# YaqiangCao/cLoops

Measured on AMD Instinct MI355X. Metric: PETs clustered/sec (whole node) + wall-clock for mode-3 eps x minPts sweep, higher is better.
Workload: dtype int32; 1 GPU; synthetic-200M-23chr-mode3 (BASELINE.json configs[3]); variant=cDBSCAN2, pets=200000000, chromosomes=23, chained_cut=True, final_cut=3871, candidate_loops=3651369, parallelism=23 chromosomes LPT-sharded over 1 GPU(s)

## Files before the change

cloops_amd/csrc/cl_table.h:

```cpp
#pragma once
#include "cl_common.h"

struct Table {
    int* count; int* minx; int* maxx; int* miny; int* maxy;
    __device__ __forceinline__ cl_box get(int k) const
    {
        cl_box b; b.min_x = minx[k]; b.max_x = maxx[k]; b.min_y = miny[k]; b.max_y = maxy[k]; b.count = count[k];
        return b;
    }
};

__device__ __forceinline__ int wave_min_i(int v) { return dpp_reduce_wave(v, OpMin()); }
__device__ __forceinline__ int wave_max_i(int v) { return dpp_reduce_wave(v, OpMax()); }

#ifndef TAB_BITS
#define TAB_BITS 9
#endif
#define TAB_H (1 << TAB_BITS)
struct TableLds { int key[TAB_H], cnt[TAB_H], mnx[TAB_H], mxx[TAB_H], mny[TAB_H], mxy[TAB_H]; };

__device__ __forceinline__ void table_lds_init(TableLds& h)
{
    for (int k = threadIdx.x; k < TAB_H; k += blockDim.x) {
        h.key[k] = -1; h.cnt[k] = 0; h.mnx[k] = INT_MAX; h.mxx[k] = INT_MIN; h.mny[k] = INT_MAX; h.mxy[k] = INT_MIN;
// ... 9 lines not shown
        h = (h + 1) & (TAB_H - 1);
    }
    return -1;
}
__device__ __forceinline__ int wave_shr1(int v) { return __builtin_amdgcn_update_dpp(v, v, 0x138, 0xf, 0xf, false); }
struct WaveRuns { int dist; bool last; };
__device__ __forceinline__ WaveRuns wave_runs(int v)
{
    const int lane = threadIdx.x & 63;
    const int prev = wave_shr1(v);
    const unsigned long long B = __ballot(lane == 0 || prev != v);
    const int start = 63 - __clzll((long long)(B & (~0ull >> (63 - lane))));
    WaveRuns r;
    r.dist = lane - start;
    r.last = lane == 63 || ((B >> (lane + 1)) & 1ull);
    return r;
}
#define SEG_STEP(ctrl, rowmask, cond, ...) seg_step_values<ctrl, rowmask>((cond), __VA_ARGS__)
template <int CTRL, int ROWMASK>
__device__ __forceinline__ void seg_step_values(bool take, int& mn0, int& mx0, int& mn1, int& mx1)
{
    const int a = min(mn0, __builtin_amdgcn_update_dpp(mn0, mn0, CTRL, ROWMASK, 0xf, false));
    const int b = max(mx0, __builtin_amdgcn_update_dpp(mx0, mx0, CTRL, ROWMASK, 0xf, false));
    const int c = min(mn1, __builtin_amdgcn_update_dpp(mn1, mn1, CTRL, ROWMASK, 0xf, false));
    const int d = max(mx1, __builtin_amdgcn_update_dpp(mx1, mx1, CTRL, ROWMASK, 0xf, false));
    mn0 = take ? a : mn0; mx0 = take ? b : mx0; mn1 = take ? c : mn1; mx1 = take ? d : mx1;
}
template <int CTRL, int ROWMASK>
__device__ __forceinline__ void seg_step_min(bool take, int& m)
{
    const int a = min(m, __builtin_amdgcn_update_dpp(m, m, CTRL, ROWMASK, 0xf, false));
    m = take ? a : m;
}
__device__ __forceinline__ void table_accumulate(const Table& t, TableLds& h, int lab, int x, int y)
{
    if (!__any(lab >= 0)) return;
    const int lane = threadIdx.x & 63;
    const WaveRuns r = wave_runs(lab);
    int mnx = x, mxx = x, mny = y, mxy = y;
    SEG_STEP(0x111, 0xf, r.dist >= 1, mnx, mxx, mny, mxy);
    SEG_STEP(0x112, 0xf, r.dist >= 2, mnx, mxx, mny, mxy);
    SEG_STEP(0x114, 0xf, r.dist >= 4, mnx, mxx, mny, mxy);
    SEG_STEP(0x118, 0xf, r.dist >= 8, mnx, mxx, mny, mxy);
    SEG_STEP(0x142, 0xa, r.dist > (lane & 15), mnx, mxx, mny, mxy);
    SEG_STEP(0x143, 0xc, r.dist > (lane & 31), mnx, mxx, mny, mxy);
    if (r.last && lab >= 0) {
        const int cm = r.dist + 1;
        const int sl = tab_slot(h.key, lab);
        if (sl >= 0) {
            atomicAdd(&h.cnt[sl], cm);
            atomicMin(&h.mnx[sl], mnx); atomicMax(&h.mxx[sl], mxx);
            atomicMin(&h.mny[sl], mny); atomicMax(&h.mxy[sl], mxy);
        } else {
            atomicAdd(&t.count[lab], cm);
            atomicMin(&t.minx[lab], mnx); atomicMax(&t.maxx[lab], mxx);
            atomicMin(&t.miny[lab], mny); atomicMax(&t.maxy[lab], mxy);
        }
    }
}
__device__ __forceinline__ void table_flush(const Table& t, TableLds& h)
{
    __syncthreads();
    for (int k = threadIdx.x; k < TAB_H; k += blockDim.x) {
        if (h.key[k] < 0) continue;
        const int L = h.key[k];
        atomicAdd(&t.count[L], h.cnt[k]);
// ... 7 lines not shown
```

cloops_amd/csrc/k_lists.hip:

```cpp
#include "cl_chrom.h"

#ifdef CLOOPS_DEVEL
#define L_ABL(bit) (g.dbg2 & (bit))
#else
#define L_ABL(bit) 0
#endif
#ifdef CLOOPS_DEVEL
__device__ unsigned long long g_lstat[32];
__device__ __forceinline__ void lstat_add(int slot, int v)
{
    int t = v;
    for (int o = 32; o > 0; o >>= 1) t += __shfl_down(t, o);
    if ((threadIdx.x & 63) == 0 && t) atomicAdd(&g_lstat[slot], (unsigned long long)t);
}
extern "C" void cl_debug_lstats(unsigned long long* out)
{
    (void)hipDeviceSynchronize();
    (void)hipMemcpyFromSymbol(out, HIP_SYMBOL(g_lstat), sizeof(g_lstat));
    unsigned long long z[32] = {0};
    (void)hipMemcpyToSymbol(HIP_SYMBOL(g_lstat), z, sizeof(z));
}
#define LSTAT_ON (g.dbg2 & (1 << 30))
#define LSTAT(slot, v) do { if (LSTAT_ON) lstat_add((slot), (v)); } while (0)
#else
// ... 377 lines not shown
        const int fin = min(m, lmin[l_hlast - t0]);
        if (threadIdx.x == 0) lmin[l_hlast - t0] = fin;
        for (int j = tend + (int)threadIdx.x; j < jend; j += 64) bkey[j] = fin;
    }
    __syncthreads();
#pragma unroll
    for (int u = 0; u < 8; ++u) {
        const int i = t0 + u * 256 + (int)threadIdx.x;
        if (i < npos && pos[u] >= t0) bkey[i] = lmin[pos[u] - t0];
    }
}

__global__ void __launch_bounds__(256)
k_words_to_base(GridParams g, int npos, const int* __restrict__ bsp, const int4* __restrict__ tab, const int* __restrict__ poff,
                const int* __restrict__ run_words, int* __restrict__ words)
{
    const int b = blockIdx.x * blockDim.x + threadIdx.x;
    if (b >= npos) return;
    const int st = min(bsp[b] >> g.rbits, g.S);
    const int4 t = tab[st];
    if (b < t.x) return;
    int w = run_words[b - poff[st]];
    if (w < 0 && ((unsigned)w & K2H_NONE) != K2H_NONE) {
        const int da = (int)((unsigned)w & K2H_MASK) + t.z, db = (int)(((unsigned)w >> K2H_BITS) & K2H_MASK) + tab[min(st + 1, g.S)].z;
        const bool ok = (da < (int)K2H_MASK) & (db < (int)K2H_MASK);
        w = (int)(((unsigned)w & ~K2H_NONE) | (ok ? ((unsigned)da | ((unsigned)db << K2H_BITS)) : K2H_NONE));
    }
    words[b] = w;
}

template <bool CUT, bool BAND>
__global__ void __launch_bounds__(256)
k_classify_q(GridParams g, int npos, int thr, int bandq, const int* __restrict__ bq, const int* __restrict__ words,
             const int* __restrict__ band, unsigned long long* __restrict__ cmask, unsigned long long* __restrict__ wmask,
             int* __restrict__ cgloc, int* __restrict__ wgloc, int* __restrict__ bsum, unsigned long long* __restrict__ sup)
{
    __shared__ int l_cc[LG], l_wc[LG];
    const int nblk = (int)gridDim.x, blk = (int)blockIdx.x;
    const int t0 = blk * LT;
    const int lane = threadIdx.x & 63, wv = threadIdx.x >> 6;
    int q[8], w[8];
#pragma unroll
    for (int u = 0; u < 8; ++u) { const int b = t0 + u * 256 + (int)threadIdx.x; q[u] = (CUT && b < npos) ? bq[b] : INT_MAX; }
#pragma unroll
    for (int u = 0; u < 8; ++u) {
        const int b = t0 + u * 256 + (int)threadIdx.x;
        const bool alive = b < npos && (!CUT || q[u] >= thr);
        const int* src = (BAND && q[u] < bandq) ? band : words;
        w[u] = alive ? src[b] : 0;
    }
#pragma unroll
    for (int u = 0; u < 8; ++u) {
        const bool core = cw_core(w[u], g.minPts) && w[u] != 0;
        const bool walk = !core && cw_count(w[u]) > 1;
        const unsigned long long cb = __ballot(core), wb = __ballot(walk);
        const int k = u * 4 + wv, gidx = (t0 >> 6) + k;
        if (lane == 0) { cmask[gidx] = cb; wmask[gidx] = wb; l_cc[k] = __popcll(cb); l_wc[k] = __popcll(wb); }
    }
    if (blk == nblk - 1 && threadIdx.x == 0) {
        const int ge = nblk * LG;
        cmask[ge] = 0ull; wmask[ge] = 0ull; cgloc[ge] = 0; wgloc[ge] = 0;
    }
    __syncthreads();
    if (threadIdx.x < 64) {
        const int k = lane & 31;
        const int v = lane < 32 ? l_cc[k] : l_wc[k];
        int incl = v;
#pragma unroll
        for (int d = 1; d < 32; d <<= 1) { const int t = __shfl_up(incl, d, 32); incl += k >= d ? t : 0; }
        (lane < 32 ? cgloc : wgloc)[(t0 >> 6) + k] = incl - v;
        const int totC = __shfl(incl, 31), totW = __shfl(incl, 63);
        if (threadIdx.x == 0 && !L_ABL(1 << 18)) {
            bsum[blk] = totC; bsum[nblk + 1 + blk] = totW;
            const unsigned long long both = (unsigned long long)(unsigned)totC | ((unsigned long long)(unsigned)totW << 32);
            if (both) atomicAdd(&sup[blk >> 4], both);
        }
    }
}

template <bool V2, bool CUT, bool BAND>
__global__ void __launch_bounds__(256)
k_make_lists_q(GridParams g, int npos, int bandq, const int* __restrict__ bq, const int* __restrict__ bsp, const u32* __restrict__ brow,
               const int* __restrict__ bkey, const int2* __restrict__ fix, const int* __restrict__ words, const int* __restrict__ band,
               const unsigned long long* __restrict__ cmask, const unsigned long long* __restrict__ wmask, const int* __restrict__ cgloc,
               const int* __restrict__ wgloc, const int* __restrict__ bsum, const unsigned long long* __restrict__ sup,
               int* __restrict__ cgrank, int* __restrict__ wgrank, int2* __restrict__ cpair, int* __restrict__ cpos,
               int* __restrict__ ckey, int2* __restrict__ wpair, int* __restrict__ wpos, int* __restrict__ wenc, int* __restrict__ lcnt,
               int* __restrict__ parent )
{
    __shared__ int l_red[2][4];
    const int nblk = (int)gridDim.x, blk = (int)blockIdx.x;
    const int t0 = blk * LT;
    const int lane = threadIdx.x & 63, wv = threadIdx.x >> 6;
    unsigned long long cbv[8], wbv[8];
    int cgv[8], wgv[8], q[8], sp[8], aux[8];
#pragma unroll
    for (int u = 0; u < 8; ++u) {
        const int gidx = (t0 >> 6) + u * 4 + wv;
        cbv[u] = cmask[gidx]; wbv[u] = wmask[gidx];
        cgv[u] = cgloc[gidx]; wgv[u] = wgloc[gidx];
        const int b = t0 + u * 256 + (int)threadIdx.x;
        q[u] = b < npos ? bq[b] : 0; sp[u] = b < npos ? bsp[b] : 0;
    }
    {
        int2 fx[8];
#pragma unroll
        for (int u = 0; u < 8; ++u) {
            const int b = t0 + u * 256 + (int)threadIdx.x;
// ... 125 lines not shown
    }
}

#define LU_MAXB 4
__device__ __forceinline__ int lower_bound_pairs(const int2* __restrict__ pv, int lo, int hi, int val)
{
    while (hi - lo > 4) {
        const int qq = (hi - lo) >> 2;
        const int m1 = lo + qq, m2 = m1 + qq, m3 = m2 + qq;
        const int v1 = pv[m1].x, v2 = pv[m2].x, v3 = pv[m3].x;
        if (v1 >= val) hi = m1;
        else if (v2 >= val) { lo = m1 + 1; hi = m2; }
        else if (v3 >= val) { lo = m2 + 1; hi = m3; }
        else lo = m3 + 1;
    }
    while (lo < hi && pv[lo].x < val) ++lo;
    return lo;
}

struct HeadReset { int* compkey; int* ncore; int* bsize; int* usize; int* state; };
template <int NT, int HALO, bool FUSE>
__global__ void __launch_bounds__(256)
k_union_c(GridParams g, int ntiles, const int* __restrict__ lcnt, const int2* __restrict__ cpair, int* chainid,
          const int* __restrict__ cstrip, int* cskip, int* parent, HeadReset hr, int* __restrict__ ckey_prune ,
          int* __restrict__ ovlist, int* __restrict__ counters)
{
    constexpr int WIN = NT + HALO;
    constexpr int NCH = WIN / 64;
    __shared__ int2 lw[WIN];
    __shared__ int lx[WIN];
    __shared__ int lend[WIN];
    __shared__ unsigned long long l_ob[FUSE ? NCH : 1];
    __shared__ int l_found;
    const int C = lcnt[0];
    const int tile = ltile_of_block(blockIdx.x);
    const int t0 = tile * NT;
    if (tile >= ntiles || t0 >= C) return;
    const int base = t0 - HALO;
    const int lane = threadIdx.x & 63;
    const int nmask = ~(g.peps - 1);
    if (FUSE && threadIdx.x == 0) l_found = -1;
    int pf_tb[NT / 256], pf_b[NT / 256];
    {
        constexpr int SU = (WIN + 255) / 256;
        static_assert(WIN % 64 == 0, "whole waves in the last staging round");
        int2 mv[SU], pvl[SU];
#pragma unroll
        for (int u = 0; u < SU; ++u) {
            const int gi = base + u * 256 + (int)threadIdx.x;
            const bool in = gi >= 0 && gi < C && u * 256 + (int)threadIdx.x < WIN;
            mv[u] = in ? cpair[gi] : (gi < 0 ? make_int2(0, INT_MIN) : make_int2(INT_MAX, INT_MAX));
            pvl[u] = (FUSE && lane == 0 && gi > 0 && gi < C) ? cpair[gi - 1] : make_int2(0, 0);
        }
        if (HALO % 256 == 0) {
#pragma unroll
            for (int u2 = 0; u2 < NT / 256; ++u2) {
                const int gi = t0 + u2 * 256 + (int)threadIdx.x;
                const int s = mv[HALO / 256 + u2].y >> g.rbits;
                const bool ok = gi < C && s > 0;
                pf_tb[u2] = ok ? cstrip[s - 1] : 0; pf_b[u2] = ok ? cstrip[s] : 0;
            }
        }
#pragma unroll
        for (int u = 0; u < SU; ++u) {
            const int k = u * 256 + (int)threadIdx.x, gi = base + k;
            if (k >= WIN) continue;
            const bool in = gi >= 0 && gi < C;
            const int2 me = mv[u];
            lw[k] = me;
            if (!FUSE) { lx[k] = in ? chainid[gi] : -1; lend[k] = in ? cskip[gi] : 0; }
            else {
                int2 pv = make_int2(wave_shr1(me.x), wave_shr1(me.y));
                if (lane == 0 && gi > 0 && gi < C) pv = pvl[u];
                const bool o = gi <= 0 ? gi == 0 : (gi >= C || (pv.y & nmask) != (me.y & nmask) || pv.x < me.x - g.eps);
                const unsigned long long ob = __ballot(o);
                if (lane == 0) l_ob[k >> 6] = ob;
            }
        }
    }
    __syncthreads();
    if (FUSE) {
        if (threadIdx.x < 64 && base > 0 && !(l_ob[0] & 1ull)) {
            int found = -1;
            for (int k0 = base - 64; found < 0; k0 -= 64) {
                const int j = k0 + lane;
                bool o = false;
                if (j >= 0) {
                    const int2 a = cpair[j];
                    const int2 b = j > 0 ? cpair[j - 1] : make_int2(0, INT_MIN);
                    o = j == 0 || (b.y & nmask) != (a.y & nmask) || b.x < a.x - g.eps;
                }
                const unsigned long long bal = __ballot(o);
                if (bal) found = k0 + 63 - __clzll((long long)bal);
            }
            if (lane == 0) l_found = found;
        }
        __syncthreads();
        for (int k = threadIdx.x; k < WIN; k += 256) {
            const int ch = k >> 6, gi = base + k;
            const unsigned long long ob = l_ob[ch];
            const unsigned long long upto = ob & (~0ull >> (63 - lane));
            int head;
            if (upto) head = base + ch * 64 + 63 - __clzll((long long)upto);
            else {
                head = l_found;
                for (int c2 = ch - 1; c2 >= 0; --c2) { const unsigned long long o2 = l_ob[c2]; if (o2) { head = base + c2 * 64 + 63 - __clzll((long long)o2); break; } }
            }
            const unsigned long long above = lane == 63 ? 0ull : (ob & (~0ull << (lane + 1)));
            int skip;
            if (above) skip = base + ch * 64 + __ffsll((long long)above) - 1;
            else {
                skip = base + WIN;
                for (int c2 = ch + 1; c2 < NCH; ++c2) { const unsigned long long o2 = l_ob[c2]; if (o2) { skip = base + c2 * 64 + __ffsll((long long)o2) - 1; break; } }
            }
            const bool in = gi >= 0 && gi < C;
            lx[k] = in ? head : -1;
            lend[k] = in ? min(skip, C) : 0;
            if (in && k >= HALO) {
                chainid[gi] = head;
                cskip[gi] = min(skip, C);
                if (head == gi) { hr.compkey[gi] = INT_MAX; hr.ncore[gi] = 0; hr.bsize[gi] = 0; hr.usize[gi] = 0; hr.state[gi] = ST_LIVE; }
                if (ckey_prune && gi > 0) {
                    const int2 me = lw[k], pv = lw[k - 1];
                    if ((pv.y & nmask) == (me.y & nmask) && div_eps(g, pv.x) == div_eps(g, me.x)) ckey_prune[gi] = INT_MAX;
                }
            }
        }
        __syncthreads();
    }
    const int wbeg = max(base, 0);
    LdsPairs w; w.a = lw; w.base = base;
    constexpr int PER = NT / 256;
#pragma unroll 1
    for (int u = 0; u < PER; ++u) {
        const int i = t0 + u * 256 + (int)threadIdx.x;
        const bool in = i < C;
        int Bs[LU_MAXB];
#pragma unroll
        for (int k = 0; k < LU_MAXB; ++k) Bs[k] = -1;
        int nb = 0;
        int A = -1;
#ifdef CLOOPS_DEVEL
        int st_it = 0, st_touch = 0, st_glb = 0, st_jump = 0;
#endif
        if (in) {
            const int2 me = lw[i - base];
            A = lx[i - base];
            const int s = me.y >> g.rbits;
            int tb, b;
            if (HALO % 256 == 0) { tb = u == 0 ? pf_tb[0] : pf_tb[NT / 256 - 1]; b = u == 0 ? pf_b[0] : pf_b[NT / 256 - 1]; }
            else { tb = s > 0 ? cstrip[s - 1] : 0; b = s > 0 ? cstrip[s] : 0; }
            if (tb < b) {
                const int qlo = me.x - g.eps, qhi = me.x + g.eps;
                const int T = me.y - g.peps;
                if (tb < wbeg && wbeg < b && lw[wbeg - base].x < qlo) tb = wbeg;
                auto touch = [&](int B) {
                    bool seen = false;
#pragma unroll
                    for (int k = 0; k < LU_MAXB; ++k) seen |= (Bs[k] == B);
                    if (seen) return;
#ifdef CLOOPS_DEVEL
                    ++st_touch;
#endif
                    if (nb < LU_MAXB) {
#pragma unroll
                        for (int k = 0; k < LU_MAXB; ++k) if (k == nb) Bs[k] = B;
                        ++nb;
                    } else {
                        uf_unite(parent, A, B);
                    }
                };
                if (L_ABL(1 << 17)) tb = b;
                if (tb >= b) { }
                else if (tb >= wbeg && b - tb <= 2047) {
                    const int len = b - tb;
                    int j;
                    if (len <= 31) j = lds_lower_bound8<5>(w, tb, b, qlo);
                    else if (len <= 63) j = lds_lower_bound8<6>(w, tb, b, qlo);
                    else if (len <= 255) j = lds_lower_bound8<8>(w, tb, b, qlo);
                    else j = lds_lower_bound8<11>(w, tb, b, qlo);
                    if (L_ABL(1 << 16)) j = b;
                    while (j < b) {
#ifdef CLOOPS_DEVEL
                        ++st_it;
#endif
                        int2 cv[4];
#pragma unroll
                        for (int k = 0; k < 4; ++k) cv[k] = lw[min(j + k, b - 1) - base];
                        int f = 4; bool fh = false;
#pragma unroll
                        for (int k = 3; k >= 0; --k) {
                            const bool bey = (j + k >= b) | (cv[k].x > qhi);
                            const bool hit = cv[k].y >= T;
                            if (bey | hit) { f = k; fh = hit & !bey; }
                        }
                        if (f == 4) { j += 4; continue; }
                        if (!fh) break;
                        const int idx = j + f - base;
                        touch(lx[idx]);
#ifdef CLOOPS_DEVEL
                        ++st_jump;
#endif
                        j = lend[idx];
                    }
                } else if (FUSE) {
                    ovlist[atomicAdd(&counters[CTR_NOVF], 1)] = i;
                } else {
#ifdef CLOOPS_DEVEL
                    ++st_glb;
#endif
                    int k = lower_bound_pairs(cpair, tb, b, qlo);
                    while (k < b) {
                        int2 cv[4]; int bv[4];
#pragma unroll
                        for (int e = 0; e < 4; ++e) { const int idx = min(k + e, b - 1); cv[e] = cpair[idx]; bv[e] = chainid[idx]; }
                        int next = k + 4;
                        bool stop = false;
#pragma unroll
                        for (int e = 0; e < 4; ++e) {
                            if (stop || k + e >= b) continue;
                            if (cv[e].x > qhi) { stop = true; next = b; continue; }
                            if (cv[e].y >= T) {
                                touch(bv[e]);
                                stop = true;
                                next = cskip[min(k + e, b - 1)];
                            }
                        }
                        k = next;
                    }
                }
            }
        }
        int st_un = 0;
#pragma unroll
        for (int k = 0; k < LU_MAXB; ++k) {
            const int B = Bs[k];
            unsigned long long pending = __ballot(B >= 0);
            bool rep = false;
            while (pending) {
                const int leader = __ffsll((long long)pending) - 1;
                const int LA = __builtin_amdgcn_readlane(A, leader), LB = __builtin_amdgcn_readlane(B, leader);
                const unsigned long long m = __ballot(B >= 0 && A == LA && B == LB);
                if (lane == leader) rep = true;
                pending &= ~m;
            }
            if (rep && !L_ABL(1 << 15)) { uf_unite(parent, A, B); ++st_un; }
        }
#ifdef CLOOPS_DEVEL
        LSTAT(12, in ? 1 : 0); LSTAT(13, st_it); LSTAT(14, st_touch); LSTAT(15, st_un); LSTAT(16, st_glb); LSTAT(17, st_jump);
        { int mx = st_it; for (int o2 = 32; o2 > 0; o2 >>= 1) mx = max(mx, __shfl_down(mx, o2)); if (lane == 0 && LSTAT_ON) { atomicAdd(&g_lstat[18], (unsigned long long)mx); atomicAdd(&g_lstat[19], 1ull); }
          if (LSTAT_ON && st_it > 2) atomicAdd(&g_lstat[20], 1ull); if (LSTAT_ON && st_it > 4) atomicAdd(&g_lstat[21], 1ull); if (LSTAT_ON && st_it > 8) atomicAdd(&g_lstat[22], 1ull); }
#else
        (void)st_un;
#endif
    }
}

__global__ void k_prep_c(GridParams g, const int* __restrict__ lcnt, const int* __restrict__ strip_start,
                         const unsigned long long* __restrict__ cmask, const int* __restrict__ cgrank, int* __restrict__ cstrip,
                         int* __restrict__ sup, int nsup2, int* __restrict__ parent )
{
    const int C = lcnt[0];
    const int u = blockIdx.x * blockDim.x + threadIdx.x;
    if (parent && u < C) parent[u] = u;
    if (u <= g.S + 1) {
        const int M = strip_start[g.S];
        const int p = u <= g.S ? strip_start[u] : M;
        cstrip[u] = p < M ? core_rank(cmask, cgrank, p) : C;
    }
    if (u < nsup2) sup[u] = 0;
}
__global__ void k_union_overflow(GridParams g, const int* __restrict__ counters, const int* __restrict__ ovlist, const int2* __restrict__ cpair,
                                 const int* __restrict__ chainid, const int* __restrict__ cstrip, const int* __restrict__ cskip, int* parent)
{
    const int nov = counters[CTR_NOVF];
    for (int t = blockIdx.x * blockDim.x + threadIdx.x; t < nov; t += gridDim.x * blockDim.x) {
        const int i = ovlist[t];
        const int2 me = cpair[i];
        const int A = chainid[i];
        const int s = me.y >> g.rbits;
        if (s <= 0) continue;
        const int tb = cstrip[s - 1], b = cstrip[s];
// ... 829 lines not shown
    c->l_sup_dirty = true;
    launch_classify(c, g, nblk, b);
    launch_make_lists(c, g, nblk, b, L);
    fuse_knob(c);
    if (c->fuse_chains)
        hipLaunchKernelGGL(k_prep_c, dim3(nblocks(std::max(std::max(nm, g.S + 2), b.nsup2))), dim3(TPB), 0, c->stream, g, (const int*)L.lcnt, (const int*)c->w_strip,
                           (const unsigned long long*)L.cmask, (const int*)L.cgrank, L.cstrip, b.sup, b.nsup2, c->parent.as<int>());
#ifdef CLOOPS_DEVEL
    else
    hipLaunchKernelGGL(k_chain_c, dim3(nblocks(nm, 256 * CH_PER)), dim3(256), 0, c->stream, g, L.lcnt, (const int2*)L.cpair, c->chainflag.as<int>(),
                       c->parent.as<int>(), c->compkey.as<int>(), c->ncore.as<int>(), c->bsize.as<int>(), c->usize.as<int>(), c->state.as<int>(),
                       c->cellfirst.as<int>() , (const int*)c->w_strip, L.cmask, L.cgrank, L.cstrip, b.sup, b.nsup2, (int*)nullptr);
#else
    { }
#endif
    L.npos = nm; L.pstrip = c->w_strip;
    *out = L;
    HIP_TRY(hipGetLastError());
    c->l_sup_dirty = false;
    return CL_OK;
}

int lists_base_keys(cl_chrom* c, const GridParams& g)
{
    const int n = (int)c->n;
    int rc = c->bkey.ensure((size_t)n * 4);
    if (rc) return rc;
    hipLaunchKernelGGL(k_base_keys, dim3(nblocks(n, LT)), dim3(256), 0, c->stream, g, n, (const int*)(c->bq.as<int>() + SORT_PAD),
                       (const int*)(c->bsp.as<int>() + SORT_PAD), (const u32*)c->brow.as<u32>(), c->bkey.as<int>());
    HIP_TRY(hipGetLastError());
    return CL_OK;
}

int lists_build_base(cl_chrom* c, const GridParams& g, int nm, ListRun* out)
{
    fuse_knob(c);
    const int n = (int)c->n;
    ListBufs b;
    int rc = list_bufs(c, g, n, &b);
    if (rc) return rc;
    const int nblk = nblocks(n, LT);
    const bool v2 = g.variant == CL_VARIANT_CDBSCAN2;
    ListRun L{};
    list_views(c, b, &L);
    L.npos = n; L.pstrip = c->bstrip.as<int>();
    unsigned long long* sup64 = (unsigned long long*)b.sup;
    const int nsup_ints = 2 * (nblk / 16 + 2);
    if (c->l_sup_dirty) HIP_TRY(hipMemsetAsync(b.sup, 0, (size_t)std::max(nsup_ints, b.nsup2) * 4, c->stream));
    c->l_sup_dirty = true;
    const int* bq = c->bq.as<int>() + SORT_PAD;
    const int* bsp = c->bsp.as<int>() + SORT_PAD;
    const u32* brow = c->brow.as<u32>();
    c->srow = c->brow.as<u32>();
    const int* words = c->rc_cnt.as<int>();
    const int* band = c->cnt.as<int>();
    const int thr = c->l4_cut ? g.cut - g.V0 : INT_MIN;
    const int bandq = c->ws.bandq;
#define LCQ_ARGS g, n, thr, bandq, bq, words, band, b.cmask, b.wmask, b.cgloc, b.wgloc, b.bsum, sup64
    if (!c->l4_cut) hipLaunchKernelGGL((k_classify_q<false, false>), dim3(nblk), dim3(256), 0, c->stream, LCQ_ARGS);
    else if (c->l4_band) hipLaunchKernelGGL((k_classify_q<true, true>), dim3(nblk), dim3(256), 0, c->stream, LCQ_ARGS);
    else hipLaunchKernelGGL((k_classify_q<true, false>), dim3(nblk), dim3(256), 0, c->stream, LCQ_ARGS);
#undef LCQ_ARGS
#define LMQ_ARGS g, n, bandq, bq, bsp, brow, (const int*)c->bkey.as<int>(), (const int2*)c->l_fix.as<int2>(), words, band, (const unsigned long long*)b.cmask,                  \
                 (const unsigned long long*)b.wmask, (const int*)b.cgloc, (const int*)b.wgloc, (const int*)b.bsum, (const unsigned long long*)sup64, b.cgrank, b.wgrank, L.cpair,  \
                 c->run_rows ? L.cpos : (int*)nullptr, L.ckey, L.wpair, L.wpos, L.wenc, b.lcnt, c->fuse_chains ? c->parent.as<int>() : (int*)nullptr
    if (v2) {
        if (!c->l4_cut) hipLaunchKernelGGL((k_make_lists_q<true, false, false>), dim3(nblk), dim3(256), 0, c->stream, LMQ_ARGS);
        else if (c->l4_band) hipLaunchKernelGGL((k_make_lists_q<true, true, true>), dim3(nblk), dim3(256), 0, c->stream, LMQ_ARGS);
        else hipLaunchKernelGGL((k_make_lists_q<true, true, false>), dim3(nblk), dim3(256), 0, c->stream, LMQ_ARGS);
    } else {
        if (c->l4_band) hipLaunchKernelGGL((k_make_lists_q<false, true, true>), dim3(nblk), dim3(256), 0, c->stream, LMQ_ARGS);
        else hipLaunchKernelGGL((k_make_lists_q<false, false, false>), dim3(nblk), dim3(256), 0, c->stream, LMQ_ARGS);
    }
#undef LMQ_ARGS
    fuse_knob(c);
    if (c->fuse_chains)
        hipLaunchKernelGGL(k_prep_c, dim3(nblocks(std::max(g.S + 2, std::max(nsup_ints, b.nsup2)))), dim3(TPB), 0, c->stream, g, (const int*)L.lcnt,
                           (const int*)L.pstrip, (const unsigned long long*)L.cmask, (const int*)L.cgrank, L.cstrip, b.sup, std::max(nsup_ints, b.nsup2), (int*)nullptr);
#ifdef CLOOPS_DEVEL
    else
    hipLaunchKernelGGL(k_chain_c, dim3(nblocks(nm, 256 * CH_PER)), dim3(256), 0, c->stream, g, L.lcnt, (const int2*)L.cpair, c->chainflag.as<int>(),
                       c->parent.as<int>(), c->compkey.as<int>(), c->ncore.as<int>(), c->bsize.as<int>(), c->usize.as<int>(), c->state.as<int>(),
                       c->cellfirst.as<int>() , L.pstrip, L.cmask, L.cgrank, L.cstrip, b.sup, std::max(nsup_ints, b.nsup2), v2 ? L.ckey : (int*)nullptr);
#else
    { }
#endif
    *out = L;
    HIP_TRY(hipGetLastError());
    c->l_sup_dirty = false;
    return CL_OK;
}

int lists_words_to_base(cl_chrom* c, const GridParams& g)
{
    const int n = (int)c->n;
// ... 182 lines not shown
    HIP_TRY(hipMemsetAsync(p + o_sup, 0, nsup * 8, c->stream));
    hipLaunchKernelGGL(k_rowmask_count, dim3((unsigned)ntile), dim3(256), 0, c->stream, (int)n, (const int*)sl.labels.as<int>(), (unsigned long long*)p,
                       (int*)(p + o_tsum), (unsigned long long*)(p + o_sup));
    hipLaunchKernelGGL(k_rowmask_write, dim3((unsigned)ntile), dim3(256), 0, c->stream, (int)n, (const int*)sl.labels.as<int>(), (const unsigned long long*)p,
                       (const int*)(p + o_tsum), (const unsigned long long*)(p + o_sup), (int*)(p + o_lab), (long long)c->mask_cap, total);
    HIP_TRY(hipGetLastError());
    return CL_OK;
}

#ifdef CLOOPS_DEVEL
extern "C" int cl_debug_time_lists(cl_chrom* c, int which, int reps, float* ms_out)
{
    if (!c || !ms_out || c->dbg_nm <= 0) return fail(CL_ERR_ARG, "cl_debug_time_lists: no rotated run on this handle");
    HIP_TRY(hipSetDevice(c->device));
    GridParams g = c->dbg_g;
    { const char* e = getenv("CLOOPS_DBG2"); g.dbg2 = e ? atoi(e) : 0; }
    const int nm = c->dbg_nm;
    ListBufs b;
    int rc = list_bufs(c, g, nm, &b);
    if (rc) return rc;
    const int nblk = nblocks(nm, LT);
    ListRun L{};
    list_views(c, b, &L);
    hipEvent_t e0, e1;
    HIP_TRY(hipEventCreate(&e0)); HIP_TRY(hipEventCreate(&e1));
    HIP_TRY(hipStreamSynchronize(c->stream));
    HIP_TRY(hipEventRecord(e0, c->stream));
    for (int r = 0; r < reps; ++r) {
        if (which == 0) {
            HIP_TRY(hipMemsetAsync(b.sup, 0, (size_t)b.nsup2 * 4, c->stream));
            launch_classify(c, g, nblk, b);
        } else if (which == 1) {
            launch_make_lists(c, g, nblk, b, L);
        } else if (which == 6 || which == 7) {
            const int n = (int)c->n;
            ListBufs bb;
            if ((rc = list_bufs(c, g, n, &bb))) return rc;
            const int nb4 = nblocks(n, LT);
            unsigned long long* sup64 = (unsigned long long*)bb.sup;
            const int* bq = c->bq.as<int>() + SORT_PAD; const int* bsp = c->bsp.as<int>() + SORT_PAD;
            const int thr = g.cut - g.V0, bandq = c->ws.bandq;
            if (which == 6) {
                HIP_TRY(hipMemsetAsync(bb.sup, 0, (size_t)2 * (nb4 / 16 + 2) * 4, c->stream));
                hipLaunchKernelGGL((k_classify_q<true, true>), dim3(nb4), dim3(256), 0, c->stream, g, n, thr, bandq, bq, (const int*)c->rc_cnt.as<int>(), (const int*)c->cnt.as<int>(),
                                   bb.cmask, bb.wmask, bb.cgloc, bb.wgloc, bb.bsum, sup64);
            } else {
                hipLaunchKernelGGL((k_make_lists_q<true, true, true>), dim3(nb4), dim3(256), 0, c->stream, g, n, bandq, bq, bsp, (const u32*)c->brow.as<u32>(), (const int*)c->bkey.as<int>(),
                                   (const int2*)c->l_fix.as<int2>(), (const int*)c->rc_cnt.as<int>(), (const int*)c->cnt.as<int>(), (const unsigned long long*)bb.cmask,
                                   (const unsigned long long*)bb.wmask, (const int*)bb.cgloc, (const int*)bb.wgloc, (const int*)bb.bsum, (const unsigned long long*)sup64, bb.cgrank, bb.wgrank,
                                   L.cpair, (int*)nullptr, L.ckey, L.wpair, L.wpos, L.wenc, bb.lcnt, (int*)nullptr);
            }
        } else if (which == 4 || which == 3 || which == 5) {
            ListRun L2 = L;
            c->run_level = c->traversal >= 4 ? 4 : 3;
            if (c->run_level == 4) { ListBufs bb; if ((rc = list_bufs(c, g, (int)c->n, &bb))) return rc; list_views(c, bb, &L2); L2.npos = (int)c->n; L2.pstrip = c->bstrip.as<int>(); }
            else { L2.npos = nm; L2.pstrip = c->w_strip; }
            if (which == 4) { if ((rc = lists_border(c, g, nm, L2))) return rc; }
            else if (which == 3) {
                ListBufs bb; if ((rc = list_bufs(c, g, c->run_level == 4 ? (int)c->n : nm, &bb))) return rc;
                fuse_knob(c);
                if (c->fuse_chains)
                    hipLaunchKernelGGL(k_prep_c, dim3(nblocks(std::max(nm, g.S + 2))), dim3(TPB), 0, c->stream, g, (const int*)L2.lcnt, (const int*)L2.pstrip,
                                       (const unsigned long long*)L2.cmask, (const int*)L2.cgrank, L2.cstrip, bb.sup, 2, c->parent.as<int>());
#ifdef CLOOPS_DEVEL
                else
                hipLaunchKernelGGL(k_chain_c, dim3(nblocks(nm, 256 * CH_PER)), dim3(256), 0, c->stream, g, L2.lcnt, (const int2*)L2.cpair, c->chainflag.as<int>(),
                                   c->parent.as<int>(), c->compkey.as<int>(), c->ncore.as<int>(), c->bsize.as<int>(), c->usize.as<int>(), c->state.as<int>(),
                                   c->cellfirst.as<int>(), L2.pstrip, L2.cmask, L2.cgrank, L2.cstrip, bb.sup, 2, (int*)nullptr);
#else
    { }
#endif
                HIP_TRY(hipMemsetAsync(c->counters.p, 0, 64, c->stream));
                if ((rc = lists_union_flatten(c, g, nm, L2))) return rc;
            } else { if ((rc = lists_final(c, g, nm, L2, false, c->counters.as<int>() + 40))) return rc; }
        } else return fail(CL_ERR_ARG, "cl_debug_time_lists: kernel not supported on its own");
    }
    HIP_TRY(hipEventRecord(e1, c->stream));
    HIP_TRY(hipEventSynchronize(e1));
    if (which == 1 || which == 7) HIP_TRY(hipMemsetAsync(b.sup, 0, c->l_blk.bytes - 64, c->stream));
    float ms = 0.f;
    (void)hipEventElapsedTime(&ms, e0, e1);
    *ms_out = ms / (float)std::max(1, reps);
    (void)hipEventDestroy(e0); (void)hipEventDestroy(e1);
    return CL_OK;
}
#endif
```

Baseline: 15.51 billion PETs/s.

## Compact union-search work list in LDS and skip dominated cores

Adds a pre-pass in k_union_c that decides for each core in the tile whether a neighbour search is needed. It packs the search bounds into a compact LDS work list, and waves then iterate densely over that list instead of over every tile slot. In the fused path it also uses segmented wave prefix/suffix minima to skip cores dominated by neighbours in the same cell. This reduces divergence and idle lanes in the search loop, at the cost of an extra pass, LDS space, atomics, and a possible correctness risk from the domination skip.

```diff
diff --git a/cloops_amd/csrc/cl_table.h b/cloops_amd/csrc/cl_table.h
--- a/cloops_amd/csrc/cl_table.h
+++ b/cloops_amd/csrc/cl_table.h
@@ -65,6 +65,45 @@
     const int a = min(m, __builtin_amdgcn_update_dpp(m, m, CTRL, ROWMASK, 0xf, false));
     m = take ? a : m;
 }
+__device__ __forceinline__ int wave_shl1(int v) { return __builtin_amdgcn_update_dpp(v, v, 0x130, 0xf, 0xf, false); }
+struct WaveSegs { int dist, rdist; };
+__device__ __forceinline__ WaveSegs wave_segs(bool open)
+{
+    const int lane = threadIdx.x & 63;
+    const unsigned long long B = __ballot(open) | 1ull;
+    const int start = 63 - __clzll((long long)(B & (~0ull >> (63 - lane))));
+    const unsigned long long above = lane == 63 ? 0ull : (B & (~0ull << (lane + 1)));
+    const int end = above ? __ffsll((long long)above) - 1 : 64;
+    WaveSegs r;
+    r.dist = lane - start;
+    r.rdist = end - 1 - lane;
+    return r;
+}
+__device__ __forceinline__ int seg_prefix_min(const WaveSegs& w, int m)
+{
+    const int lane = threadIdx.x & 63;
+    seg_step_min<0x111, 0xf>(w.dist >= 1, m);
+    seg_step_min<0x112, 0xf>(w.dist >= 2, m);
+    seg_step_min<0x114, 0xf>(w.dist >= 4, m);
+    seg_step_min<0x118, 0xf>(w.dist >= 8, m);
+    seg_step_min<0x142, 0xa>(w.dist > (lane & 15), m);
+    seg_step_min<0x143, 0xc>(w.dist > (lane & 31), m);
+    return m;
+}
+__device__ __forceinline__ int seg_suffix_min(const WaveSegs& w, int m)
+{
+    const int lane = threadIdx.x & 63;
+    seg_step_min<0x101, 0xf>(w.rdist >= 1, m);
+    seg_step_min<0x102, 0xf>(w.rdist >= 2, m);
+    seg_step_min<0x104, 0xf>(w.rdist >= 4, m);
+    seg_step_min<0x108, 0xf>(w.rdist >= 8, m);
+#pragma unroll
+    for (int r = 3; r >= 1; --r) {
+        const int v = __builtin_amdgcn_readlane(m, 16 * r);
+        m = ((lane >> 4) == r - 1 && w.rdist > 15 - (lane & 15)) ? min(m, v) : m;
+    }
+    return m;
+}
 __device__ __forceinline__ void table_accumulate(const Table& t, TableLds& h, int lab, int x, int y)
 {
     if (!__any(lab >= 0)) return;
diff --git a/cloops_amd/csrc/k_lists.hip b/cloops_amd/csrc/k_lists.hip
--- a/cloops_amd/csrc/k_lists.hip
+++ b/cloops_amd/csrc/k_lists.hip
@@ -666,6 +666,10 @@
     __shared__ int lend[WIN];
     __shared__ unsigned long long l_ob[FUSE ? NCH : 1];
     __shared__ int l_found;
+    __shared__ unsigned lsv[NT];
+    __shared__ int l_ns;
+    constexpr int PER = NT / 256;
+    static_assert(NT <= 512 && WIN <= 1024, "a list entry packs the core's offset in the tile and its window in the staged range");
     const int C = lcnt[0];
     const int tile = ltile_of_block(blockIdx.x);
     const int t0 = tile * NT;
@@ -673,8 +677,8 @@
     const int base = t0 - HALO;
     const int lane = threadIdx.x & 63;
     const int nmask = ~(g.peps - 1);
-    if (FUSE && threadIdx.x == 0) l_found = -1;
-    int pf_tb[NT / 256], pf_b[NT / 256];
+    if (threadIdx.x == 0) { l_found = -1; l_ns = 0; }
+    int pf_tb[PER], pf_b[PER];
     {
         constexpr int SU = (WIN + 255) / 256;
         static_assert(WIN % 64 == 0, "whole waves in the last staging round");
@@ -713,6 +717,49 @@
         }
     }
     __syncthreads();
+    const int wbeg = max(base, 0);
+    {
+        int tbv[PER], bv[PER];
+#pragma unroll
+        for (int u2 = 0; u2 < PER; ++u2) {
+            if (HALO % 256 == 0) { tbv[u2] = pf_tb[u2]; bv[u2] = pf_b[u2]; }
+            else {
+                const int k = HALO + u2 * 256 + (int)threadIdx.x;
+                const int s = lw[k].y >> g.rbits;
+                const bool ok = base + k < C && s > 0;
+                tbv[u2] = ok ? cstrip[s - 1] : 0; bv[u2] = ok ? cstrip[s] : 0;
+            }
+        }
+#pragma unroll
+        for (int u2 = 0; u2 < PER; ++u2) {
+            const int k = HALO + u2 * 256 + (int)threadIdx.x, gi = base + k;
+            const bool in = gi < C;
+            const int2 me = lw[k];
+            bool dom = false;
+            if (FUSE) {
+                const int px = wave_shr1(me.x), py = wave_shr1(me.y);
+                const WaveSegs sg = wave_segs(!in || (py & nmask) != (me.y & nmask) || div_eps(g, px) != div_eps(g, me.x));
+                const int fmin = wave_shr1(seg_prefix_min(sg, me.y)), bmin = wave_shl1(seg_suffix_min(sg, me.y));
+                dom = sg.dist >= 1 && fmin <= me.y && sg.rdist >= 1 && bmin < me.y;
+            }
+            int tb = tbv[u2];
+            const int b = bv[u2];
+            bool srch = in && !dom && tb < b && !L_ABL(1 << 17);
+            if (srch && tb < wbeg && wbeg < b && lw[wbeg - base].x < me.x - g.eps) tb = wbeg;
+            const bool staged = tb >= wbeg && b - tb <= 2047;
+            LSTAT(12, in ? 1 : 0); LSTAT(23, srch ? 1 : 0);
+            if (FUSE && srch && !staged) {
+                ovlist[atomicAdd(&counters[CTR_NOVF], 1)] = gi;
+                srch = false;
+            }
+            const unsigned long long sb = __ballot(srch);
+            int wb = 0;
+            if (lane == 0 && sb) wb = atomicAdd(&l_ns, __popcll(sb));
+            wb = __builtin_amdgcn_readfirstlane(wb);
+            if (srch) lsv[wb + lane_rank(sb)] = (unsigned)(k - HALO) | (staged ? ((unsigned)(tb - base) << 9) | ((unsigned)(b - base) << 19) : 0x80000000u);
+        }
+    }
+    if (!FUSE) __syncthreads();
     if (FUSE) {
         if (threadIdx.x < 64 && base > 0 && !(l_ob[0] & 1ull)) {
             int found = -1;
@@ -762,13 +809,11 @@
         }
         __syncthreads();
     }
-    const int wbeg = max(base, 0);
     LdsPairs w; w.a = lw; w.base = base;
-    constexpr int PER = NT / 256;
+    const int ns = l_ns;
 #pragma unroll 1
-    for (int u = 0; u < PER; ++u) {
-        const int i = t0 + u * 256 + (int)threadIdx.x;
-        const bool in = i < C;
+    for (int n0 = (int)threadIdx.x - lane; n0 < ns; n0 += 256) {
+        const bool in = n0 + lane < ns;
         int Bs[LU_MAXB];
 #pragma unroll
         for (int k = 0; k < LU_MAXB; ++k) Bs[k] = -1;
@@ -778,16 +823,14 @@
         int st_it = 0, st_touch = 0, st_glb = 0, st_jump = 0;
 #endif
         if (in) {
-            const int2 me = lw[i - base];
-            A = lx[i - base];
-            const int s = me.y >> g.rbits;
-            int tb, b;
-            if (HALO % 256 == 0) { tb = u == 0 ? pf_tb[0] : pf_tb[NT / 256 - 1]; b = u == 0 ? pf_b[0] : pf_b[NT / 256 - 1]; }
-            else { tb = s > 0 ? cstrip[s - 1] : 0; b = s > 0 ? cstrip[s] : 0; }
-            if (tb < b) {
+            const unsigned ent = lsv[n0 + lane];
+            const int k0 = HALO + (int)(ent & 511u);
+            const bool staged = !(ent >> 31);
+            const int2 me = lw[k0];
+            A = lx[k0];
+            {
                 const int qlo = me.x - g.eps, qhi = me.x + g.eps;
                 const int T = me.y - g.peps;
-                if (tb < wbeg && wbeg < b && lw[wbeg - base].x < qlo) tb = wbeg;
                 auto touch = [&](int B) {
                     bool seen = false;
 #pragma unroll
@@ -804,9 +847,8 @@
                         uf_unite(parent, A, B);
                     }
                 };
-                if (L_ABL(1 << 17)) tb = b;
-                if (tb >= b) { }
-                else if (tb >= wbeg && b - tb <= 2047) {
+                if (staged) {
+                    const int tb = base + (int)((ent >> 9) & 1023u), b = base + (int)((ent >> 19) & 1023u);
                     const int len = b - tb;
                     int j;
                     if (len <= 31) j = lds_lower_bound8<5>(w, tb, b, qlo);
@@ -837,12 +879,12 @@
 #endif
                         j = lend[idx];
                     }
-                } else if (FUSE) {
-                    ovlist[atomicAdd(&counters[CTR_NOVF], 1)] = i;
-                } else {
+                } else if (!FUSE) {
 #ifdef CLOOPS_DEVEL
                     ++st_glb;
 #endif
+                    const int s = me.y >> g.rbits;
+                    const int tb = cstrip[s - 1], b = cstrip[s];
                     int k = lower_bound_pairs(cpair, tb, b, qlo);
                     while (k < b) {
                         int2 cv[4]; int bv[4];
@@ -881,7 +923,7 @@
             if (rep && !L_ABL(1 << 15)) { uf_unite(parent, A, B); ++st_un; }
         }
 #ifdef CLOOPS_DEVEL
-        LSTAT(12, in ? 1 : 0); LSTAT(13, st_it); LSTAT(14, st_touch); LSTAT(15, st_un); LSTAT(16, st_glb); LSTAT(17, st_jump);
+        LSTAT(13, st_it); LSTAT(14, st_touch); LSTAT(15, st_un); LSTAT(16, st_glb); LSTAT(17, st_jump);
         { int mx = st_it; for (int o2 = 32; o2 > 0; o2 >>= 1) mx = max(mx, __shfl_down(mx, o2)); if (lane == 0 && LSTAT_ON) { atomicAdd(&g_lstat[18], (unsigned long long)mx); atomicAdd(&g_lstat[19], 1ull); }
           if (LSTAT_ON && st_it > 2) atomicAdd(&g_lstat[20], 1ull); if (LSTAT_ON && st_it > 4) atomicAdd(&g_lstat[21], 1ull); if (LSTAT_ON && st_it > 8) atomicAdd(&g_lstat[22], 1ull); }
 #else
```

Result: no change. 15.46 billion PETs/s (-0.3%).

## Split walker classification into a pass that drops walkers seeing no core

Applied to the files above, without the earlier changes.

Core classification and walker classification now run as two kernels. The new walker kernel marks a border candidate as a walker only if a core point lies within eps in an adjacent strip. It checks this with a shared-memory copy of the core bitmask plus a halo, and falls back to a global bitmask search when the halo is not enough. The aim is to shrink the walker lists that later list-building and union stages must process, at the cost of an extra launch, extra bitmask/bq/bsp reads and possible divergence on the slow path.

```diff
diff --git a/cloops_amd/csrc/k_lists.hip b/cloops_amd/csrc/k_lists.hip
--- a/cloops_amd/csrc/k_lists.hip
+++ b/cloops_amd/csrc/k_lists.hip
@@ -433,10 +433,10 @@
 template <bool CUT, bool BAND>
 __global__ void __launch_bounds__(256)
 k_classify_q(GridParams g, int npos, int thr, int bandq, const int* __restrict__ bq, const int* __restrict__ words,
-             const int* __restrict__ band, unsigned long long* __restrict__ cmask, unsigned long long* __restrict__ wmask,
-             int* __restrict__ cgloc, int* __restrict__ wgloc, int* __restrict__ bsum, unsigned long long* __restrict__ sup)
-{
-    __shared__ int l_cc[LG], l_wc[LG];
+             const int* __restrict__ band, unsigned long long* __restrict__ cmask, int* __restrict__ cgloc, int* __restrict__ bsum,
+             unsigned long long* __restrict__ sup)
+{
+    __shared__ int l_cc[LG];
     const int nblk = (int)gridDim.x, blk = (int)blockIdx.x;
     const int t0 = blk * LT;
     const int lane = threadIdx.x & 63, wv = threadIdx.x >> 6;
@@ -453,28 +453,224 @@
 #pragma unroll
     for (int u = 0; u < 8; ++u) {
         const bool core = cw_core(w[u], g.minPts) && w[u] != 0;
-        const bool walk = !core && cw_count(w[u]) > 1;
-        const unsigned long long cb = __ballot(core), wb = __ballot(walk);
+        const unsigned long long cb = __ballot(core);
         const int k = u * 4 + wv, gidx = (t0 >> 6) + k;
-        if (lane == 0) { cmask[gidx] = cb; wmask[gidx] = wb; l_cc[k] = __popcll(cb); l_wc[k] = __popcll(wb); }
+        if (lane == 0) { cmask[gidx] = cb; l_cc[k] = __popcll(cb); }
     }
     if (blk == nblk - 1 && threadIdx.x == 0) {
         const int ge = nblk * LG;
-        cmask[ge] = 0ull; wmask[ge] = 0ull; cgloc[ge] = 0; wgloc[ge] = 0;
+        cmask[ge] = 0ull; cgloc[ge] = 0;
     }
     __syncthreads();
-    if (threadIdx.x < 64) {
-        const int k = lane & 31;
-        const int v = lane < 32 ? l_cc[k] : l_wc[k];
+    if (threadIdx.x < 32) {
+        const int k = lane;
+        const int v = l_cc[k];
         int incl = v;
 #pragma unroll
         for (int d = 1; d < 32; d <<= 1) { const int t = __shfl_up(incl, d, 32); incl += k >= d ? t : 0; }
-        (lane < 32 ? cgloc : wgloc)[(t0 >> 6) + k] = incl - v;
-        const int totC = __shfl(incl, 31), totW = __shfl(incl, 63);
+        cgloc[(t0 >> 6) + k] = incl - v;
+        const int totC = __shfl(incl, 31, 32);
         if (threadIdx.x == 0 && !L_ABL(1 << 18)) {
-            bsum[blk] = totC; bsum[nblk + 1 + blk] = totW;
-            const unsigned long long both = (unsigned long long)(unsigned)totC | ((unsigned long long)(unsigned)totW << 32);
-            if (both) atomicAdd(&sup[blk >> 4], both);
+            bsum[blk] = totC;
+            if (totC) atomicAdd(&sup[blk >> 4], (unsigned long long)(unsigned)totC);
+        }
+    }
+}
+
+__device__ __forceinline__ int first_core_in(const unsigned long long* __restrict__ cmask, int from, int end)
+{
+    if (from >= end) return end;
+    int gi = from >> 6;
+    const int ge = (end - 1) >> 6;
+    unsigned long long m = cmask[gi] & ~low_mask(from & 63);
+    while (!m && gi < ge) m = cmask[++gi];
+    return m ? min((gi << 6) + __ffsll((long long)m) - 1, end) : end;
+}
+__device__ __forceinline__ int last_core_in(const unsigned long long* __restrict__ cmask, int beg, int to)
+{
+    if (to <= beg) return -1;
+    int gi = (to - 1) >> 6;
+    const int gb = beg >> 6;
+    unsigned long long m = cmask[gi] & (((to - 1) & 63) == 63 ? ~0ull : low_mask(to & 63));
+    while (!m && gi > gb) m = cmask[--gi];
+    if (!m) return -1;
+    const int p = (gi << 6) + 63 - __clzll((long long)m);
+    return p >= beg ? p : -1;
+}
+__device__ __forceinline__ int lower_bound_q(const int* __restrict__ bq, int lo, int hi, int val)
+{
+    while (lo < hi) { const int mid = (int)(((unsigned)lo + (unsigned)hi) >> 1); if (bq[mid] < val) lo = mid + 1; else hi = mid; }
+    return lo;
+}
+__device__ __noinline__ bool walker_sees_core(int rbits, int S, int eps, int b, int q, int sp, int w, const int* __restrict__ bq,
+                                              const int* __restrict__ bsp, const int* __restrict__ bstrip, const unsigned long long* __restrict__ cmask)
+{
+    const int s = min(sp >> rbits, S - 1), peps = 1 << rbits;
+    const int qlo = q - eps, qhi = q + eps;
+    const int pbeg = sp & ~(peps - 1), pend = pbeg + peps, pend2 = pend + peps;
+    const int sb0 = bstrip[s], sb1 = bstrip[s + 1], sb2 = bstrip[min(s + 2, S)];
+    const unsigned enc = lh_pack(w, 0, 0);
+    const bool hinted = enc != LH_NONE;
+    bool keep = false;
+    const int pl = last_core_in(cmask, sb0, b);
+    if (pl >= 0) keep = (bsp[pl] >= pbeg) & (bq[pl] >= qlo);
+    if (!keep) {
+        const int pr = first_core_in(cmask, b + 1, sb1);
+        if (pr < sb1) keep = (bsp[pr] < pend) & (bq[pr] <= qhi);
+    }
+    if (!keep && s > 0) {
+        const int pa = hinted ? b - (int)(enc & 0xffffu) : lower_bound_q(bq, bstrip[s - 1], sb0, qlo);
+        const int pc = first_core_in(cmask, max(pa, 0), b);
+        if (pc < b) keep = (bsp[pc] < pbeg) & (bq[pc] <= qhi);
+    }
+    if (!keep) {
+        const int pb = hinted ? b + (int)(enc >> 16) : lower_bound_q(bq, sb1, sb2, qlo);
+        const int pc = first_core_in(cmask, pb, sb2);
+        if (pc < sb2) keep = (bsp[pc] < pend2) & (bq[pc] <= qhi);
+    }
+    return keep;
+}
+#define WQ_HALO 4096
+#define WQ_NW ((LT + 2 * WQ_HALO) / 64)
+template <bool CUT, bool BAND>
+__global__ void __launch_bounds__(256)
+k_walkers_q(GridParams g, int npos, int thr, int bandq, const int* __restrict__ bq, const int* __restrict__ bsp,
+            const int* __restrict__ bstrip, const int* __restrict__ words, const int* __restrict__ band,
+            const unsigned long long* __restrict__ cmask, unsigned long long* __restrict__ wmask, int* __restrict__ wgloc,
+            int* __restrict__ bsum, unsigned long long* __restrict__ sup)
+{
+    static_assert(WQ_NW <= 192 && (int)K2H_MASK < WQ_HALO, "three words of non-empty bits; a hint stays inside the halo");
+    __shared__ int l_wc[LG];
+    __shared__ unsigned long long l_cm[WQ_NW];
+    __shared__ unsigned long long l_nz[3];
+    const int nblk = (int)gridDim.x, blk = (int)blockIdx.x;
+    const int t0 = blk * LT;
+    const int lane = threadIdx.x & 63, wv = threadIdx.x >> 6;
+    const int gw0 = (t0 - WQ_HALO) >> 6;
+    const int wlo = max(t0 - WQ_HALO, 0), wend = min(t0 + LT + WQ_HALO, nblk * LT);
+    int q[8], w[8], sp[8];
+#pragma unroll
+    for (int u = 0; u < 8; ++u) { const int b = t0 + u * 256 + (int)threadIdx.x; q[u] = b < npos ? bq[b] : INT_MAX; }
+    {
+        const int k = (int)threadIdx.x, gw = gw0 + k;
+        const unsigned long long v = (k < WQ_NW && gw >= 0 && gw < nblk * LG) ? cmask[gw] : 0ull;
+        if (k < WQ_NW) l_cm[k] = v;
+        const unsigned long long nz = __ballot(v != 0ull);
+        if (lane == 0 && wv < 3) l_nz[wv] = nz;
+    }
+    const int sp_lo = bsp[wlo], sp_hi = bsp[min(wend, npos) - 1];
+    const bool at_front = wlo == 0, at_back = wend >= npos;
+#pragma unroll
+    for (int u = 0; u < 8; ++u) {
+        const int b = t0 + u * 256 + (int)threadIdx.x;
+        const bool alive = b < npos && (!CUT || q[u] >= thr);
+        const int* src = (BAND && q[u] < bandq) ? band : words;
+        w[u] = alive ? src[b] : 0;
+    }
+    int ncls = 0;
+#pragma unroll
+    for (int u = 0; u < 8; ++u) {
+        const int b = t0 + u * 256 + (int)threadIdx.x;
+        const bool core = cw_core(w[u], g.minPts) && w[u] != 0;
+        const bool walk = !core && cw_count(w[u]) > 1;
+        sp[u] = walk ? bsp[b] : 0;
+        if (!walk) w[u] = 0;
+        ncls += walk ? 1 : 0;
+    }
+    LSTAT(23, ncls);
+    (void)ncls;
+    __syncthreads();
+    auto next_core = [&](int from, int end) -> int {
+        if (from >= end) return -1;
+        int k = (from >> 6) - gw0;
+        if (k >= WQ_NW) return -1;
+        unsigned long long m = l_cm[k] & ~low_mask(from & 63);
+        if (!m) {
+            const int kk = k + 1;
+            int k2 = -1;
+#pragma unroll
+            for (int j = 2; j >= 0; --j) {
+                const unsigned long long mm = l_nz[j] & (j == (kk >> 6) ? ~low_mask(kk & 63) : (j > (kk >> 6) ? ~0ull : 0ull));
+                if (mm) k2 = j * 64 + __ffsll((long long)mm) - 1;
+            }
+            if (k2 < 0) return -1;
+            k = k2; m = l_cm[k2];
+        }
+        const int p = ((gw0 + k) << 6) + __ffsll((long long)m) - 1;
+        return p < end ? p : -1;
+    };
+    auto prev_core = [&](int beg, int to) -> int {
+        if (to <= beg) return -1;
+        const int last = to - 1;
+        int k = (last >> 6) - gw0;
+        unsigned long long m = l_cm[k] & ((last & 63) == 63 ? ~0ull : low_mask((last & 63) + 1));
+        if (!m) {
+            const int kk = k - 1;
+            if (kk < 0) return -1;
+            int k2 = -1;
+#pragma unroll
+            for (int j = 0; j < 3; ++j) {
+                const unsigned long long upto = (kk & 63) == 63 ? ~0ull : low_mask((kk & 63) + 1);
+                const unsigned long long mm = l_nz[j] & (j == (kk >> 6) ? upto : (j < (kk >> 6) ? ~0ull : 0ull));
+                if (mm) k2 = j * 64 + 63 - __clzll((long long)mm);
+            }
+            if (k2 < 0) return -1;
+            k = k2; m = l_cm[k2];
+        }
+        const int p = ((gw0 + k) << 6) + 63 - __clzll((long long)m);
+        return p >= beg ? p : -1;
+    };
+    int slow = 0;
+#pragma unroll
+    for (int u = 0; u < 8; ++u) {
+        const int b = t0 + u * 256 + (int)threadIdx.x;
+        const bool walk = w[u] != 0;
+        bool keep = false;
+        if (__ballot(walk)) {
+            const unsigned enc = lh_pack(w[u], 0, 0);
+            const bool hinted = enc != LH_NONE;
+            const int pa = b - (int)(enc & 0xffffu), pb = b + (int)(enc >> 16);
+            const int pl = walk ? prev_core(wlo, b) : -1;
+            const int pr = walk ? next_core(b + 1, wend) : -1;
+            const int pc = (walk && hinted && pa >= wlo) ? next_core(pa, b) : -1;
+            const int pd = (walk && hinted) ? next_core(pb, wend) : -1;
+            const int bs = min(b, npos - 1);
+            const int il = pl >= 0 ? pl : bs, ir = pr >= 0 ? pr : bs, ic = pc >= 0 ? pc : bs, id = pd >= 0 ? pd : bs;
+            const int ql = bq[il], qr = bq[ir], qc = bq[ic], qd = bq[id];
+            const int sl = bsp[il], sr = bsp[ir], sc = bsp[ic], sd = bsp[id];
+            const int qlo = q[u] - g.eps, qhi = q[u] + g.eps;
+            const int pbeg = sp[u] & ~(g.peps - 1), pend = pbeg + g.peps, pend2 = pend + g.peps;
+            keep = walk & (((pl >= 0) & (sl >= pbeg) & (ql >= qlo)) | ((pr >= 0) & (sr < pend) & (qr <= qhi)) |
+                           ((pc >= 0) & (sc < pbeg) & (qc <= qhi)) | ((pd >= 0) & (sd < pend2) & (qd <= qhi)));
+            const bool open_l = (pl < 0) & !(at_front | (sp_lo < pbeg));
+            const bool open_r = (pr < 0) & !(at_back | (sp_hi >= pend));
+            const bool open_d = (pd < 0) & !(at_back | (sp_hi >= pend2));
+            if (walk & !keep & (!hinted | (pa < wlo) | open_l | open_r | open_d)) slow |= 1 << u;
+        }
+        if (__any(slow >> u & 1)) {
+            if (slow >> u & 1) keep = walker_sees_core(g.rbits, g.S, g.eps, b, q[u], sp[u], w[u], bq, bsp, bstrip, cmask);
+            LSTAT(24, slow >> u & 1);
+        }
+        const unsigned long long wb = __ballot(keep);
+        const int k = u * 4 + wv, gidx = (t0 >> 6) + k;
+        if (lane == 0) { wmask[gidx] = wb; l_wc[k] = __popcll(wb); }
+    }
+    if (blk == nblk - 1 && threadIdx.x == 0) {
+        const int ge = nblk * LG;
+        wmask[ge] = 0ull; wgloc[ge] = 0;
+    }
+    __syncthreads();
+    if (threadIdx.x < 32) {
+        const int k = lane;
+        const int v = l_wc[k];
+        int incl = v;
+#pragma unroll
+        for (int d = 1; d < 32; d <<= 1) { const int t = __shfl_up(incl, d, 32); incl += k >= d ? t : 0; }
+        wgloc[(t0 >> 6) + k] = incl - v;
+        const int totW = __shfl(incl, 31, 32);
+        if (threadIdx.x == 0 && !L_ABL(1 << 18)) {
+            bsum[nblk + 1 + blk] = totW;
+            if (totW) atomicAdd(&sup[blk >> 4], (unsigned long long)(unsigned)totW << 32);
         }
     }
 }
@@ -1777,6 +1973,29 @@
     return CL_OK;
 }
 
+static void launch_classify_q(cl_chrom* c, const GridParams& g, int n, int nblk, int thr, int bandq, const ListBufs& b, bool cores, bool walkers)
+{
+    const int* bq = c->bq.as<int>() + SORT_PAD;
+    const int* bsp = c->bsp.as<int>() + SORT_PAD;
+    const int* words = c->rc_cnt.as<int>();
+    const int* band = c->cnt.as<int>();
+    unsigned long long* sup64 = (unsigned long long*)b.sup;
+#define LCQ_ARGS g, n, thr, bandq, bq, words, band, b.cmask, b.cgloc, b.bsum, sup64
+#define LWQ_ARGS g, n, thr, bandq, bq, bsp, (const int*)c->bstrip.as<int>(), words, band, (const unsigned long long*)b.cmask, b.wmask, b.wgloc, b.bsum, sup64
+    if (!c->l4_cut) {
+        if (cores) hipLaunchKernelGGL((k_classify_q<false, false>), dim3(nblk), dim3(256), 0, c->stream, LCQ_ARGS);
+        if (walkers) hipLaunchKernelGGL((k_walkers_q<false, false>), dim3(nblk), dim3(256), 0, c->stream, LWQ_ARGS);
+    } else if (c->l4_band) {
+        if (cores) hipLaunchKernelGGL((k_classify_q<true, true>), dim3(nblk), dim3(256), 0, c->stream, LCQ_ARGS);
+        if (walkers) hipLaunchKernelGGL((k_walkers_q<true, true>), dim3(nblk), dim3(256), 0, c->stream, LWQ_ARGS);
+    } else {
+        if (cores) hipLaunchKernelGGL((k_classify_q<true, false>), dim3(nblk), dim3(256), 0, c->stream, LCQ_ARGS);
+        if (walkers) hipLaunchKernelGGL((k_walkers_q<true, false>), dim3(nblk), dim3(256), 0, c->stream, LWQ_ARGS);
+    }
+#undef LCQ_ARGS
+#undef LWQ_ARGS
+}
+
 int lists_build_base(cl_chrom* c, const GridParams& g, int nm, ListRun* out)
 {
     fuse_knob(c);
@@ -1801,11 +2020,7 @@
     const int* band = c->cnt.as<int>();
     const int thr = c->l4_cut ? g.cut - g.V0 : INT_MIN;
     const int bandq = c->ws.bandq;
-#define LCQ_ARGS g, n, thr, bandq, bq, words, band, b.cmask, b.wmask, b.cgloc, b.wgloc, b.bsum, sup64
-    if (!c->l4_cut) hipLaunchKernelGGL((k_classify_q<false, false>), dim3(nblk), dim3(256), 0, c->stream, LCQ_ARGS);
-    else if (c->l4_band) hipLaunchKernelGGL((k_classify_q<true, true>), dim3(nblk), dim3(256), 0, c->stream, LCQ_ARGS);
-    else hipLaunchKernelGGL((k_classify_q<true, false>), dim3(nblk), dim3(256), 0, c->stream, LCQ_ARGS);
-#undef LCQ_ARGS
+    launch_classify_q(c, g, n, nblk, thr, bandq, b, true, true);
 #define LMQ_ARGS g, n, bandq, bq, bsp, brow, (const int*)c->bkey.as<int>(), (const int2*)c->l_fix.as<int2>(), words, band, (const unsigned long long*)b.cmask,                  \
                  (const unsigned long long*)b.wmask, (const int*)b.cgloc, (const int*)b.wgloc, (const int*)b.bsum, (const unsigned long long*)sup64, b.cgrank, b.wgrank, L.cpair,  \
                  c->run_rows ? L.cpos : (int*)nullptr, L.ckey, L.wpair, L.wpos, L.wenc, b.lcnt, c->fuse_chains ? c->parent.as<int>() : (int*)nullptr
@@ -2054,7 +2269,7 @@
             launch_classify(c, g, nblk, b);
         } else if (which == 1) {
             launch_make_lists(c, g, nblk, b, L);
-        } else if (which == 6 || which == 7) {
+        } else if (which == 6 || which == 7 || which == 8) {
             const int n = (int)c->n;
             ListBufs bb;
             if ((rc = list_bufs(c, g, n, &bb))) return rc;
@@ -2064,8 +2279,9 @@
             const int thr = g.cut - g.V0, bandq = c->ws.bandq;
             if (which == 6) {
                 HIP_TRY(hipMemsetAsync(bb.sup, 0, (size_t)2 * (nb4 / 16 + 2) * 4, c->stream));
-                hipLaunchKernelGGL((k_classify_q<true, true>), dim3(nb4), dim3(256), 0, c->stream, g, n, thr, bandq, bq, (const int*)c->rc_cnt.as<int>(), (const int*)c->cnt.as<int>(),
-                                   bb.cmask, bb.wmask, bb.cgloc, bb.wgloc, bb.bsum, sup64);
+                launch_classify_q(c, g, n, nb4, thr, bandq, bb, true, false);
+            } else if (which == 8) {
+                launch_classify_q(c, g, n, nb4, thr, bandq, bb, false, true);
             } else {
                 hipLaunchKernelGGL((k_make_lists_q<true, true, true>), dim3(nb4), dim3(256), 0, c->stream, g, n, bandq, bq, bsp, (const u32*)c->brow.as<u32>(), (const int*)c->bkey.as<int>(),
                                    (const int2*)c->l_fix.as<int2>(), (const int*)c->rc_cnt.as<int>(), (const int*)c->cnt.as<int>(), (const unsigned long long*)bb.cmask,
@@ -2099,7 +2315,7 @@
     }
     HIP_TRY(hipEventRecord(e1, c->stream));
     HIP_TRY(hipEventSynchronize(e1));
-    if (which == 1 || which == 7) HIP_TRY(hipMemsetAsync(b.sup, 0, c->l_blk.bytes - 64, c->stream));
+    if (which == 1 || which == 7 || which == 8) HIP_TRY(hipMemsetAsync(b.sup, 0, c->l_blk.bytes - 64, c->stream));
     float ms = 0.f;
     (void)hipEventElapsedTime(&ms, e0, e1);
     *ms_out = ms / (float)std::max(1, reps);
```

After: 15.23 billion PETs/s before, 14.36 billion PETs/s after. -5.7%, worse.
